# oviniciuscesar/Pseudo-Quadrature-Mirror-Filter

Measured on NVIDIA B200. Metric: PQMF analyze+inverse throughput (n_band=16), higher is better.
Workload: dtype f32

## Files before the change

pseudo-quadrature-mirror-filter_b200/csrc/hankel4.cuh:

```cuda
#pragma once
#include <cuda_fp16.h>
#include <cuda_runtime.h>
#include <math.h>
#include <stdint.h>
#include <string.h>

#include <atomic>

#include "half_io.cuh"
#include "hankel16.cuh"
#include "pcm.cuh"
#include "ptx.cuh"

namespace pqmf {

constexpr int kH4Workers = 256;
constexpr int kH4Threads = kH4Workers + 32;
constexpr int kH4SynWorkers = 288;
constexpr int kH4SynThreads = kH4SynWorkers + 32;
constexpr int kH4Rows = 128;
constexpr int kH4TileSamples = 64 * kH4Rows;
constexpr int kH4MaxPlaneRows = 144;
constexpr float kH4Res = 2048.0f;

// ... 39 lines not shown
  constexpr uint32_t idesc128 = ptx::umma_idesc_f16(m, 128), idesc64 = ptx::umma_idesc_f16(m, 64);
  constexpr uint32_t kStep = 2 * kBankRows;
  auto a_step = [&](int s) {
    const uint32_t byte = 32u * (uint32_t)s + (uint32_t)pad_bytes;
    return (uint64_t)(8u * (byte >> 7) + ((byte >> 4) & 7u));
  };
  auto mma = [&](uint32_t d, uint64_t a, uint64_t bdesc, uint32_t idesc, bool acc) {
    if constexpr (PAIR) ptx::umma_pair_f16(d, a, bdesc, idesc, acc);
    else ptx::umma_f16(d, a, bdesc, idesc, acc);
  };
  for (int s = tlo; s < ks - thi; ++s) mma(d_tmem, da1 + a_step(s), db + (uint64_t)(kStep * s), idesc128, s != tlo);
  for (int s = 0; s < tlo; ++s) mma(d_tmem, da1 + a_step(s), db64 + (uint64_t)(kStep * s), idesc64, true);
  for (int s = ks - thi; s < ks; ++s) mma(d_tmem, da1 + a_step(s), db64 + (uint64_t)(kStep * s), idesc64, true);
  for (int s = tlo; s < ks - thi; ++s) mma(d_tmem + 64u, da2 + a_step(s), db64 + (uint64_t)(kStep * s), idesc64, true);
}

__device__ __forceinline__ void split2_f16s(float a, float b, uint32_t& h1_bits, uint32_t& h2_bits) {
  const __half2 h1 = __floats2half2_rn(a, b);
  const float2 h1f = __half22float2(h1);
  const float2 r = __ffma2_rn(h1f, make_float2(-kH4Res, -kH4Res), __fmul2_rn(make_float2(a, b), make_float2(kH4Res, kH4Res)));
  const __half2 h2 = __floats2half2_rn(r.x, r.y);
  h1_bits = *reinterpret_cast<const uint32_t*>(&h1);
  h2_bits = *reinterpret_cast<const uint32_t*>(&h2);
}
__device__ __forceinline__ float2 h4_combine2(uint32_t d0a, uint32_t d0b, uint32_t d1a, uint32_t d1b) {
  const float2 t = __ffma2_rn(make_float2(__uint_as_float(d1a), __uint_as_float(d1b)), make_float2(1.0f / kH4Res, 1.0f / kH4Res),
                              make_float2(__uint_as_float(d0a), __uint_as_float(d0b)));
  constexpr float kInv = 1.0f / (float)(1 << kH16ScaleLog2);
  return __fmul2_rn(t, make_float2(kInv, kInv));
}

template <int N>
__device__ __forceinline__ void h4_tmem_ld(uint32_t taddr, uint32_t (&r)[N]) {
  static_assert(N == 2 || N == 4 || N == 8 || N == 16 || N == 32, "columns per load");
  if constexpr (N == 2) ptx::tmem_ld2(taddr, r);
  else if constexpr (N == 4) ptx::tmem_ld4(taddr, r);
  else if constexpr (N == 8) ptx::tmem_ld8(taddr, r);
  else if constexpr (N == 16) ptx::tmem_ld16(taddr, r);
  else ptx::tmem_ld32(taddr, r);
}

__device__ __forceinline__ void h4_split_store8(const float (&w)[8], unsigned char* p1, int plane, uint32_t off) {
  uint4 a, bq;
  split2_f16s(w[0], w[1], a.x, bq.x);
  split2_f16s(w[2], w[3], a.y, bq.y);
  split2_f16s(w[4], w[5], a.z, bq.z);
  split2_f16s(w[6], w[7], a.w, bq.w);
  unsigned char* p2 = p1 + plane;
  *reinterpret_cast<uint4*>(p1 + off) = a;
  *reinterpret_cast<uint4*>(p2 + off) = bq;
}

__device__ __forceinline__ void h4_synthesis_chunk8(const float4 (&v)[8], int j, uint32_t fl, float (&w)[8]) {
#pragma unroll
  for (int kk = 0; kk < 8; ++kk) {
    const float t = j == 0 ? v[kk].x : j == 1 ? v[kk].y : j == 2 ? v[kk].z : v[kk].w;
    w[kk] = (kk & 1) ? __uint_as_float(__float_as_uint(t) ^ fl) : t;
  }
}

template <int M>
__device__ __forceinline__ void h4_drain_analysis(uint32_t tmem, int dbuf, int tid, int first, int parity, float (&v)[64 / M][M / 2]) {
  constexpr int FR = 64 / M, HB = M / 2;
  const uint32_t taddr = tmem + ((uint32_t)(((tid >> 5) & 3) * 32) << 16) + (uint32_t)(dbuf * 128 + HB * (tid >> 7));
  uint32_t r0[FR][HB], r1[FR][HB];
#pragma unroll
  for (int dl = 0; dl < FR; ++dl) {
    h4_tmem_ld<HB>(taddr + dl * M, r0[dl]);
    h4_tmem_ld<HB>(taddr + 64 + dl * M, r1[dl]);
  }
  ptx::tmem_ld_wait();
#pragma unroll
  for (int dl = 0; dl < FR; ++dl) {
    const uint32_t flip = (((FR > 1 ? dl : first) + parity) & 1) == 0 ? 0x80000000u : 0u;
#pragma unroll
    for (int kk = 0; kk < HB; kk += 2) {
      const float2 t = h4_combine2(r0[dl][kk], r0[dl][kk + 1], r1[dl][kk], r1[dl][kk + 1]);
      v[dl][kk] = t.x;
      v[dl][kk + 1] = __uint_as_float(__float_as_uint(t.y) ^ flip);
    }
  }
}

__device__ __forceinline__ void h4_drain_synthesis(uint32_t tmem, int dbuf, int tid, float (&val)[4][8]) {
  const int hb = tid >> 7, lane = tid & 31;
  const uint32_t taddr = tmem + ((uint32_t)(((tid >> 5) & 3) * 32) << 16) + (uint32_t)(dbuf * 128 + 2 * hb * 16);
  uint32_t r0[2][16], r1[2][16];
  ptx::tmem_ld16(taddr, r0[0]);
  ptx::tmem_ld16(taddr + 64, r1[0]);
  ptx::tmem_ld16(taddr + 16, r0[1]);
  ptx::tmem_ld16(taddr + 80, r1[1]);
  ptx::tmem_ld_wait();
#pragma unroll
  for (int q = 0; q < 4; ++q)
#pragma unroll
    for (int e = 0; e < 8; e += 2) {
      const int c0 = 8 * (q & 1) + e;
      const float2 t = h4_combine2(r0[q >> 1][c0], r0[q >> 1][c0 + 1], r1[q >> 1][c0], r1[q >> 1][c0 + 1]);
      val[q][e] = t.x;
      val[q][e + 1] = t.y;
    }
  const bool b0 = lane & 1, b1 = lane & 2;
#pragma unroll
  for (int pr = 0; pr < 2; ++pr)
#pragma unroll
    for (int e = 0; e < 8; ++e) {
      const float recv = __shfl_xor_sync(0xffffffffu, b0 ? val[2 * pr][e] : val[2 * pr + 1][e], 1);
      val[2 * pr + 1][e] = b0 ? val[2 * pr + 1][e] : recv;
      val[2 * pr][e] = b0 ? recv : val[2 * pr][e];
    }
#pragma unroll
  for (int u = 0; u < 2; ++u)
#pragma unroll
    for (int e = 0; e < 8; ++e) {
      const float recv = __shfl_xor_sync(0xffffffffu, b1 ? val[u][e] : val[u + 2][e], 2);
      val[u + 2][e] = b1 ? val[u + 2][e] : recv;
      val[u][e] = b1 ? recv : val[u][e];
    }
}

#ifdef PQMF_H4_TRACE
#define H4_TRACE_PARAM , long long* trace
#define H4_TRACE(x) , x
#define H4_STAMP(k) do { if (trace && blockIdx.x == 0 && (tid & 31) == 0 && it < 64) trace[((size_t)it * 8 + (tid >> 5)) * 8 + (k)] = clock64(); } while (0)
#else
#define H4_TRACE_PARAM
#define H4_TRACE(x)
#define H4_STAMP(k) do { } while (0)
#endif

struct H4Smem {
  unsigned char *bank, *planes;
  uint64_t *pfull, *mma_bar, *bankfull;
  uint32_t* tmem_slot;
};
__device__ __forceinline__ H4Smem h4_carve(unsigned char* smem, const H4Shape& g) {
  H4Smem s;
  s.bank = smem;
  s.planes = smem + g.bank;
  s.pfull = reinterpret_cast<uint64_t*>(smem + g.bank + 4 * g.plane);
  s.mma_bar = s.pfull + 2;
  s.bankfull = s.mma_bar + 2;
  s.tmem_slot = reinterpret_cast<uint32_t*>(s.bankfull + 1);
  return s;
}

template <bool PAIR>
__device__ __forceinline__ uint32_t h4_prologue(const H4Smem& s, const H4Shape& g, const uint16_t* bank_images, uint32_t rank, int worker_warps,
                                                int tid) {
  const int warp = tid >> 5;
  ptx::grid_dep_launch();
  if (tid == 0) {
    for (int i = 0; i < 2; ++i) {
      ptx::mbar_init(&s.pfull[i], worker_warps * (PAIR ? 2 : 1));
      ptx::mbar_init(&s.mma_bar[i], 1);
    }
    ptx::mbar_init(s.bankfull, 1);
    ptx::fence_barrier_init();
    ptx::mbar_arrive_expect_tx(s.bankfull, (uint32_t)g.bank);
    ptx::bulk_g2s(s.bank, reinterpret_cast<const unsigned char*>(bank_images) + (size_t)rank * g.bank, (uint32_t)g.bank, s.bankfull);
  }
  if (warp == 0) {
    if constexpr (PAIR) {
      ptx::tmem_alloc_pair(s.tmem_slot, 256);
    } else {
      ptx::tmem_alloc(s.tmem_slot, 256);
      ptx::tmem_relinquish();
    }
  }
  ptx::tc_fence_before();
  __syncthreads();
  if constexpr (PAIR) ptx::cluster_sync_all();
  ptx::tc_fence_after();
  ptx::grid_dep_wait();
  return *s.tmem_slot;
}

template <bool PAIR>
__device__ __forceinline__ void h4_teardown(uint32_t tmem, int warp) {
  ptx::tc_fence_before();
  __syncthreads();
  if constexpr (PAIR) {
    ptx::cluster_sync_all();
    if (warp == 0) ptx::tmem_dealloc_pair(tmem, 256);
  } else {
    if (warp == 0) ptx::tmem_dealloc(tmem, 256);
  }
}

template <bool PAIR>
__device__ __forceinline__ void h4_issuer_loop(const H4Smem& s, const H4Shape& g, uint32_t tmem, unsigned n_iter, int pad_bytes, int tlo,
                                               int thi) {
  const uint32_t bank_addr = ptx::smem_u32(s.bank), plane_addr = ptx::smem_u32(s.planes);
  for (unsigned it = 0; it < n_iter; ++it) {
    const int pb = (int)(it & 1);
    ptx::mbar_wait(&s.pfull[pb], (it >> 1) & 1);
    ptx::tc_fence_after();
    if (ptx::elect_one_sync()) {
      h4_issue_mmas<PAIR>(tmem + (uint32_t)(pb * 128), plane_addr + (2 * pb) * g.plane, plane_addr + (2 * pb + 1) * g.plane, bank_addr, g.ks,
                          pad_bytes, tlo, thi);
// ... 296 lines not shown
    const int n_fq = (g.rows * FR + FPI - 1) / FPI;
    const int bg = tid / n_fq, fq = tid - bg * n_fq;
    const bool has_item = tid < n_fq * NBG;
    float4 v0[8];
    auto load4h = [&](const uint16_t* at, bool ok) {
      if (!ok) return make_float4(0.f, 0.f, 0.f, 0.f);
      const float2 raw = ptx::ldg64_na(at);
      return make_float4(raw.x, raw.y, 0.f, 0.f);
    };
    auto load_frames = [&](unsigned bb, unsigned cc, unsigned hh) {
      if (p.reverse && bb < n_rows) {
        bb = n_rows - 1 - bb;
        cc = tpr - 1 - cc;
      }
      const long n = (long)cc * (kH4Rows * FR) + nbase + FPI * fq;
      const bool live = bb < n_rows && has_item;
      const size_t row = (size_t)bb * G + hh;
      if constexpr (HALF) {
        if constexpr (M >= 8) {
          const uint16_t* sp = reinterpret_cast<const uint16_t*>(p.s) + (row * M + 8 * bg) * p.F + n;
          const bool ok = live && n >= 0 && n + 3 < p.F;
#pragma unroll
          for (int kk = 0; kk < 8; ++kk) v0[kk] = load4h(sp + (size_t)kk * p.F, ok);
        } else {
          const uint16_t* sp = reinterpret_cast<const uint16_t*>(p.s) + row * M * p.F + n;
#pragma unroll
          for (int kk = 0; kk < 8; ++kk) {
            const int b4 = kk >> 1, hf = kk & 1;
            v0[kk] = load4h(sp + (size_t)b4 * p.F + 4 * hf, live && n + 4 * hf >= 0 && n + 4 * hf + 3 < p.F);
          }
        }
      } else if constexpr (M >= 8) {
        const float* sp = p.s + (row * M + 8 * bg) * p.F + n;
        const bool ok = live && n >= 0 && n + 3 < p.F;
#pragma unroll
        for (int kk = 0; kk < 8; ++kk) v0[kk] = ok ? ptx::ldg128_na(reinterpret_cast<const float4*>(sp + (size_t)kk * p.F)) : make_float4(0.f, 0.f, 0.f, 0.f);
      } else {
        const float* sp = p.s + row * M * p.F + n;
#pragma unroll
        for (int kk = 0; kk < 8; ++kk) {
          const int b4 = kk >> 1, hf = kk & 1;
          const bool ok = live && n + 4 * hf >= 0 && n + 4 * hf + 3 < p.F;
          v0[kk] = ok ? ptx::ldg128_na(reinterpret_cast<const float4*>(sp + (size_t)b4 * p.F + 4 * hf)) : make_float4(0.f, 0.f, 0.f, 0.f);
        }
      }
    };
    const uint32_t flip_even = (p.parity & 1) ? 0u : 0x80000000u, flip_odd = flip_even ^ 0x80000000u;
    auto convert = [&](int pb) {
      float4 v[8];
#pragma unroll
      for (int kk = 0; kk < 8; ++kk) v[kk] = HALF ? h4_widen4<IO>(v0[kk]) : v0[kk];
      if (!has_item) return;
      unsigned char* p1 = sm.planes + (2 * pb) * g.plane;
#pragma unroll
      for (int j = 0; j < 4; ++j) {
        float w[8];
        uint32_t o;
        if constexpr (M >= 8) {
          h4_synthesis_chunk8(v, j, (j & 1) ? flip_odd : flip_even, w);
          o = sw128_offset((uint32_t)(4 * fq + j) * (2u * M) + 16u * bg);
        } else {
#pragma unroll
          for (int kk = 0; kk < 8; ++kk) {
            const int b4 = kk & 3, odd = kk >> 2;
            const float4& q = v[2 * b4 + (j >> 1)];
            const int cmp = 2 * (j & 1) + odd;
            const float t = cmp == 0 ? q.x : cmp == 1 ? q.y : cmp == 2 ? q.z : q.w;
            w[kk] = (b4 & 1) ? __uint_as_float(__float_as_uint(t) ^ (odd ? flip_odd : flip_even)) : t;
          }
          o = sw128_offset((uint32_t)(8 * fq + 2 * j) * (2u * M));
        }
        h4_split_store8(w, p1, g.plane, o);
      }
    };
    uint32_t held[4][4];
    auto drain = [&](int dbuf) {
      if (warp >= 8 || prev_b >= n_rows) return;
      unsigned bb = prev_b, cc = prev_c;
      if (p.reverse) {
        bb = n_rows - 1 - bb;
        cc = tpr - 1 - cc;
      }
      const size_t row = (size_t)bb * G + prev_h;
      const int i = tid & 127, hb = tid >> 7, lane = tid & 31;
      float val[4][8];
      h4_drain_synthesis(tmem, dbuf, tid, val);
      const long total = p.F * M;
      const long t0 = (long)cc * kH4TileSamples + 64 * (i & ~3) + 32 * hb + 8 * (lane & 3);
      if constexpr (PCM) {
        if (G == 2) {
#pragma unroll
          for (int q = 0; q < 4; ++q) {
            uint32_t w[4];
#pragma unroll
            for (int k = 0; k < 4; ++k)
              w[k] = (uint32_t)(uint16_t)pcm_quantise(val[q][2 * k]) | ((uint32_t)(uint16_t)pcm_quantise(val[q][2 * k + 1]) << 16);
            if (prev_h == 0) {
#pragma unroll
              for (int k = 0; k < 4; ++k) held[q][k] = w[k];
            } else if (t0 + 64 * q + 7 < total) {
              float lr[8];
#pragma unroll
              for (int k = 0; k < 4; ++k) {
                lr[2 * k] = __uint_as_float(__byte_perm(held[q][k], w[k], 0x5410));
                lr[2 * k + 1] = __uint_as_float(__byte_perm(held[q][k], w[k], 0x7632));
              }
              ptx::stg256_cs(reinterpret_cast<float*>(p.pcm_out + ((size_t)bb * total + t0 + 64 * q) * 2), lr);
            }
          }
          return;
        }
#pragma unroll
        for (int q = 0; q < 4; ++q)
          if (t0 + 64 * q + 7 < total) pcm_store8(p.pcm_out, p.C, (long)row, t0 + 64 * q, total, val[q]);
        return;
      }
      if constexpr (HALF) {
        uint16_t* op = reinterpret_cast<uint16_t*>(p.out) + row * total + t0;
#pragma unroll
        for (int q = 0; q < 4; ++q)
          if (t0 + 64 * q + 7 < total) {
            const uint4 w = make_uint4(h4_narrow2<IO>(val[q][0], val[q][1]), h4_narrow2<IO>(val[q][2], val[q][3]), h4_narrow2<IO>(val[q][4], val[q][5]),
                                       h4_narrow2<IO>(val[q][6], val[q][7]));
            __stcs(reinterpret_cast<uint4*>(op + (size_t)q * 64), w);
          }
        return;
      }
      float* op = p.out + row * total + t0;
#pragma unroll
      for (int q = 0; q < 4; ++q)
        if (t0 + 64 * q + 7 < total) {
          if (p.accumulate) {
            float prev[8];
            ptx::ldg256_cs(op + (size_t)q * 64, prev);
#pragma unroll
            for (int e = 0; e < 8; ++e) val[q][e] += prev[e];
          }
          ptx::stg256_cs(op + (size_t)q * 64, val[q]);
        }
    };

    load_frames(b, c, h);
    h4_worker_loop<PAIR>(sm, pfull_leader, n_iter, tid, convert, [&] { load_frames(b1, c1, h1); }, drain, [&] {
      prev_b = b;
      prev_c = c;
      prev_h = h;
      b = b1;
      c = c1;
      h = h1;
      next_visit(b1, c1, h1);
    } H4_TRACE(p.trace));
  } H4_TRACE(p.trace));
}

struct H4Configured {
  std::atomic<int> bytes[64];
  H4Configured() {
    for (auto& b : bytes) b.store(0, std::memory_order_relaxed);
  }
};
inline int h4_sm_count(int dev) {
  static std::atomic<int> sm_count[64];
  int n = sm_count[dev].load(std::memory_order_relaxed);
  if (n == 0) {
    cudaDeviceGetAttribute(&n, cudaDevAttrMultiProcessorCount, dev);
    n = n > 0 ? n : 148;
    sm_count[dev].store(n, std::memory_order_relaxed);
  }
  return n;
}
template <typename Kern>
inline int h4_configure(Kern kern, int bytes, H4Configured& configured, int& sm_count_out) {
  int dev = 0;
  cudaGetDevice(&dev);
  dev &= 63;
  if (configured.bytes[dev].load(std::memory_order_acquire) < bytes) {
    cudaError_t e = cudaFuncSetAttribute(kern, cudaFuncAttributeMaxDynamicSharedMemorySize, bytes);
    if (e != cudaSuccess) return (int)e;
    int seen = configured.bytes[dev].load(std::memory_order_relaxed);
    while (seen < bytes && !configured.bytes[dev].compare_exchange_weak(seen, bytes, std::memory_order_release)) {
    }
  }
  sm_count_out = h4_sm_count(dev);
  return 0;
}

template <typename Params>
inline bool h4_set_tiles(Params& p, int B, long row_samples) {
  p.tiles_per_row = (row_samples + kH4TileSamples - 1) / kH4TileSamples;
  p.n_tiles = p.tiles_per_row * B;
  return p.tiles_per_row < (1L << 31) && p.n_tiles < (1L << 40);
}

template <bool PAIR, typename Kern, typename Params>
inline int h4_launch(Kern kern, const Params& p, int threads, H4Configured& configured, cudaStream_t st) {
  int sms = 0;
  if (!h4_shape_fits(p.g)) return -2;
  if (int e = h4_configure(kern, p.g.bytes, configured, sms)) return e;
  long grid = PAIR ? (sms & ~1) : sms;
  const long want = PAIR ? ((p.n_tiles + 1) & ~1L) : p.n_tiles;
  if (grid > want) grid = want;
  if constexpr (PAIR) {
    cudaLaunchConfig_t cfg = {};
    cfg.gridDim = dim3((unsigned)grid);
    cfg.blockDim = dim3((unsigned)threads);
    cfg.dynamicSmemBytes = (size_t)p.g.bytes;
    cfg.stream = st;
    cudaLaunchAttribute attr[2];
    attr[0].id = cudaLaunchAttributeClusterDimension;
    attr[0].val.clusterDim.x = 2;
    attr[0].val.clusterDim.y = 1;
    attr[0].val.clusterDim.z = 1;
    attr[1].id = cudaLaunchAttributeProgrammaticStreamSerialization;
    attr[1].val.programmaticStreamSerializationAllowed = 1;
    cfg.attrs = attr;
    cfg.numAttrs = 2;
    return (int)cudaLaunchKernelEx(&cfg, kern, p);
  } else {
    kern<<<(unsigned)grid, threads, p.g.bytes, st>>>(p);
    return (int)cudaGetLastError();
  }
}

template <int M, bool PAIR>
int h4_launch_analysis(H4AnalysisParams p, int B, cudaStream_t st, H4Io io = H4Io::F32) {
  static H4Configured configured[4];
  if (!h4_set_tiles(p, B, p.F * M)) return -2;
  if (p.in.pcm != nullptr) io = H4Io::PCM;
  if (io != H4Io::F32) {
    if constexpr (PAIR) {
      switch (io) {
        case H4Io::PCM: return h4_launch<PAIR>(h4_analysis_kernel<M, PAIR, H4Io::PCM>, p, kH4Threads, configured[1], st);
        case H4Io::F16: return h4_launch<PAIR>(h4_analysis_kernel<M, PAIR, H4Io::F16>, p, kH4Threads, configured[2], st);
        case H4Io::BF16: return h4_launch<PAIR>(h4_analysis_kernel<M, PAIR, H4Io::BF16>, p, kH4Threads, configured[3], st);
        default: return -2;
      }
    } else {
      return -2;
    }
  }
  return h4_launch<PAIR>(h4_analysis_kernel<M, PAIR, H4Io::F32>, p, kH4Threads, configured[0], st);
}

template <int M, bool PAIR>
int h4_launch_synthesis(H4SynthesisParams p, int B, cudaStream_t st, H4Io io = H4Io::F32) {
  static H4Configured configured[4];
  if (p.pcm_out != nullptr) {
    if constexpr (PAIR) {
      p.duo = (p.C == 2 && B % 2 == 0) ? 1 : 0;
      if (!h4_set_tiles(p, p.duo ? B / 2 : B, p.F * M)) return -2;
      return h4_launch<PAIR>(h4_synthesis_kernel<M, PAIR, H4Io::PCM>, p, kH4SynThreads, configured[1], st);
    } else {
      return -2;
    }
  }
  if (!h4_set_tiles(p, B, p.F * M)) return -2;
  if (h4_io_half(io)) {
    if constexpr (PAIR) {
      if (io == H4Io::F16) return h4_launch<PAIR>(h4_synthesis_kernel<M, PAIR, H4Io::F16>, p, kH4SynThreads, configured[2], st);
      return h4_launch<PAIR>(h4_synthesis_kernel<M, PAIR, H4Io::BF16>, p, kH4SynThreads, configured[3], st);
    } else {
      return -2;
    }
  }
  return h4_launch<PAIR>(h4_synthesis_kernel<M, PAIR, H4Io::F32>, p, kH4SynThreads, configured[0], st);
}

inline void hankel4_build_banks(const float* hk , int M, int L, int jlo, int kt, uint16_t* img_analysis, uint16_t* img_synthesis) {
  auto bits = [](float v) {
    const __half h = __float2half_rn(v);
    uint16_t u;
    memcpy(&u, &h, 2);
    return u;
  };
  const int ks = (kt + 64 - M + 15) / 16, kp = 16 * ks;
  const int elo = jlo / M, ehi = (jlo + kt) / M - 1;
  const float sa = (float)(1 << kH16ScaleLog2), ss = (float)M * sa;
  for (int kc = 0; kc < kp / 8; ++kc)
    for (int row = 0; row < 128; ++row)
      for (int e8 = 0; e8 < 8; ++e8) {
        const int kap = 8 * kc + e8;
        const int part = row / 64, delta = (row % 64) / M, q = row % M;
        const size_t at = ((size_t)kc * 128 + row) * 8 + e8;
        {
          const int j = kap - M * delta;
          const float v = (j >= 0 && j < kt && jlo + j < L) ? sa * hk[(size_t)q * L + jlo + j] : 0.f;
          const float c1 = __half2float(__float2half_rn(v));
          img_analysis[at] = part == 0 ? bits(c1) : bits((v - c1) * kH4Res);
        }
        {
          const int e = kap / M, kb = kap % M, lag = delta + ehi - e;
          const float v = (lag >= elo && lag <= ehi && M * lag + q < L) ? ss * hk[(size_t)kb * L + M * lag + q] : 0.f;
          const float c1 = __half2float(__float2half_rn(v));
          img_synthesis[at] = part == 0 ? bits(c1) : bits((v - c1) * kH4Res);
        }
      }
}

inline void hankel4_pair_image(const uint16_t* single , int ks, uint16_t* pair ) {
  const int chunks = 2 * ks;
  for (int r = 0; r < 2; ++r)
    for (int kc = 0; kc < chunks; ++kc)
      for (int row = 0; row < 96; ++row) {
        const int src = row < 64 ? 64 * r + row : 32 * r + (row - 64);
        memcpy(pair + (((size_t)r * chunks + kc) * 96 + row) * 8, single + ((size_t)kc * 128 + src) * 8, 16);
      }
}

inline int hankel4_pick_trim(const float* hk , int M, int L, int jlo, int kt, bool synthesis, double budget, int max_trim = 7) {
  const int ks = (kt + 64 - M + 15) / 16, fr = 64 / M, elo = jlo / M, ehi = (jlo + kt) / M - 1;
  int best = 0;
  for (int trim = 1; trim <= max_trim && ks - 2 * trim >= 1; ++trim) {
    double worst = 0.0;
    for (int delta = 0; delta < fr; ++delta)
      for (int q = 0; q < M; ++q) {
        double sum = 0.0;
        for (int side = 0; side < 2; ++side)
          for (int t = 0; t < trim; ++t) {
            const int s = side ? ks - 1 - t : t;
            for (int e16 = 0; e16 < 16; ++e16) {
              const int kap = 16 * s + e16;
              if (!synthesis) {
                const int j = kap - M * delta;
                if (j >= 0 && j < kt && jlo + j < L) sum += fabs((double)hk[(size_t)q * L + jlo + j]);
              } else {
                const int e = kap / M, kb = kap % M, lag = delta + ehi - e;
                if (lag >= elo && lag <= ehi && M * lag + q < L) sum += (double)M * fabs((double)hk[(size_t)kb * L + M * lag + q]);
              }
            }
          }
        worst = sum > worst ? sum : worst;
      }
    if (2.0 * worst / 2048.0 <= budget) best = trim;
    else break;
  }
  return best;
}

}
```

pseudo-quadrature-mirror-filter_b200/csrc/hankel4_stream.cuh:

```cuda
#pragma once
#include <type_traits>

#include "hankel4.cuh"
#include "stream_pool.cuh"

namespace pqmf {

struct H4StreamGeom {
  int rows_b;
  int hrows;
  int pitch;
  int spt;
};
inline H4StreamGeom h4_stream_geom(long block_samples, int hist_samples) {
  H4StreamGeom s;
  s.rows_b = (int)(block_samples / 64);
  s.hrows = hist_samples / 64;
  s.pitch = (s.rows_b + s.hrows + 3) & ~3;
  s.spt = kH4Rows / s.pitch;
  return s;
}

struct H4AnalysisStreamParams {
  const float* x;
// ... 195 lines not shown
    const int tid = threadIdx.x, warp = tid >> 5;
    for (int u = sg.spt * sg.pitch * 32 + tid; u < g.rows * 32; u += kH4SynWorkers)
#pragma unroll
      for (int pl = 0; pl < 4; ++pl) reinterpret_cast<float*>(sm.planes + pl * g.plane)[u] = 0.f;
    const int n_fq = sg.spt * sg.pitch * FR / 4;
    const int bg = tid / n_fq, wq = tid - bg * n_fq;
    const bool has_item = tid < NBG * n_fq;
    const int region_frames = sg.pitch * FR, hist_fr = sg.hrows * FR, block_fr = sg.rows_b * FR;
    const int lt = (4 * wq) / region_frames, lf = 4 * wq - lt * region_frames;
    const int fb = lf - hist_fr;
    constexpr int kDead = 1 << 20;
    const size_t band0 = ((size_t)blockIdx.x * sg.spt + lt) * M + 8 * bg;
    const size_t step_state = (size_t)gridDim.x * sg.spt * M * p.K;
    int slot = kDead;
    const float* src = p.s;
    size_t src_step = 0, src_pitch = 0;
    float* roll = nullptr;
    int hofs = -1, rofs = -1;
    if (has_item) {
      if (fb < 0) {
        slot = lt;
        if constexpr (POOL) {
          hofs = 8 * bg * p.K + (p.K - hist_fr) + lf;
        } else {
          src = p.state_in + band0 * p.K + (p.K - hist_fr) + lf;
          src_step = step_state;
        }
        src_pitch = (size_t)p.K;
      } else if (fb < block_fr) {
        slot = lt;
        src = p.s + band0 * p.F + fb;
        src_step = (size_t)gridDim.x * sg.spt * M * p.F;
        src_pitch = (size_t)p.F;
        if (fb >= p.F - p.K) {
          if constexpr (POOL) rofs = 8 * bg * p.K + (fb - (p.F - p.K));
          else roll = p.state_out + band0 * p.K + (fb - (p.F - p.K));
        }
      }
    }
    float4 v[8];
    int nlive = 0;
    uint32_t flip_ld = 0;
    auto load_tile = [&](long tile) {
      nlive = (int)min((long)sg.spt, (long)p.B - tile * sg.spt);
      if constexpr (POOL) {
        int id = slot < nlive ? __ldg(p.pool.ids + tile * sg.spt + slot) : -1;
        if ((unsigned)id >= (unsigned)p.pool.P) id = -1;
        const int ph = id >= 0 ? __ldg(p.pool.phase + id) : 0;
        const size_t row = ((size_t)(ph & 1) * p.pool.P + (size_t)id) * M * p.K;
        const float* from = hofs >= 0 ? p.state_in + row + hofs : src;
#pragma unroll
        for (int kk = 0; kk < 8; ++kk)
          v[kk] = id >= 0 ? ptx::ldg128_na(reinterpret_cast<const float4*>(from + (size_t)kk * src_pitch)) : make_float4(0.f, 0.f, 0.f, 0.f);
        src += src_step;
        roll = (rofs >= 0 && id >= 0) ? p.state_out + ((size_t)(~ph & 1) * p.pool.P + (size_t)id) * M * p.K + rofs : nullptr;
        flip_ld = (ph & 2) ? 0u : 0x80000000u;
      } else {
        const bool live = slot < nlive;
#pragma unroll
        for (int kk = 0; kk < 8; ++kk)
          v[kk] = live ? ptx::ldg128_na(reinterpret_cast<const float4*>(src + (size_t)kk * src_pitch)) : make_float4(0.f, 0.f, 0.f, 0.f);
        src += src_step;
      }
    };
    const uint32_t flip_even = (p.parity & 1) ? 0u : 0x80000000u, flip_odd = flip_even ^ 0x80000000u;
    auto convert = [&](int pb) {
      if (!has_item) return;
      unsigned char* p1 = sm.planes + (2 * pb) * g.plane;
      const uint32_t fe = POOL ? flip_ld : flip_even, fo = POOL ? flip_ld ^ 0x80000000u : flip_odd;
      if (roll != nullptr) {
        if (POOL || slot < nlive) {
#pragma unroll
          for (int kk = 0; kk < 8; ++kk) *reinterpret_cast<float4*>(roll + (size_t)kk * p.K) = v[kk];
        }
        if constexpr (!POOL) roll += step_state;
      }
#pragma unroll
      for (int j = 0; j < 4; ++j) {
        float w[8];
        h4_synthesis_chunk8(v, j, (j & 1) ? fo : fe, w);
        h4_split_store8(w, p1, g.plane, sw128_offset((uint32_t)(4 * wq + j) * (2u * M) + 16u * bg));
      }
    };
    const int i = tid & 127, hb = tid >> 7, lane = tid & 31;
    const int i0 = i & ~3, et = i0 / sg.pitch, eq0 = i0 - et * sg.pitch;
    const bool e_rows = et < sg.spt && eq0 < sg.rows_b;
    float* orun = p.out + ((size_t)blockIdx.x * sg.spt + et) * (size_t)(p.F * M) + 64 * eq0 + 32 * hb + 8 * (lane & 3);
    const size_t out_step = (size_t)gridDim.x * sg.spt * (size_t)(p.F * M);
    long tile = blockIdx.x, prev_tile = 0;
    auto drain = [&](int dbuf) {
      if (warp >= 8) return;
      float val[4][8];
      h4_drain_synthesis(tmem, dbuf, tid, val);
      float* op = orun;
      orun += out_step;
      if (!e_rows || prev_tile * sg.spt + et >= p.B) return;
#pragma unroll
      for (int q = 0; q < 4; ++q) ptx::stg256_cs(op + (size_t)q * 64, val[q]);
    };

    load_tile(tile);
    h4_worker_loop<true>(sm, pfull_leader, n_iter, tid, convert, [&] { load_tile(tile + gridDim.x); }, drain, [&] {
      prev_tile = tile;
      tile += gridDim.x;
    } H4_TRACE(nullptr));
  } H4_TRACE(nullptr));
}

template <int M, typename Params>
inline int h4_launch_analysis_stream(Params p, cudaStream_t st) {
  constexpr bool POOL = std::is_same_v<Params, H4AnalysisStreamPoolParams>;
  static H4Configured configured;
  p.n_tiles = (p.B + p.s.spt - 1) / p.s.spt;
  return h4_launch<true>(h4_analysis_stream_kernel<M, POOL>, p, kH4Threads, configured, st);
}
template <int M, typename Params>
inline int h4_launch_synthesis_stream(Params p, cudaStream_t st) {
  constexpr bool POOL = std::is_same_v<Params, H4SynthesisStreamPoolParams>;
  static H4Configured configured;
  p.n_tiles = (p.B + p.sg.spt - 1) / p.sg.spt;
  return h4_launch<true>(h4_synthesis_stream_kernel<M, POOL>, p, kH4SynThreads, configured, st);
}

}
```

pseudo-quadrature-mirror-filter_b200/csrc/ptx.cuh:

```cuda
#pragma once
#include <cuda_fp16.h>
#include <cuda_runtime.h>
#include <stdint.h>

namespace pqmf {
namespace ptx {

__device__ __forceinline__ uint32_t smem_u32(const void* p) { return (uint32_t)__cvta_generic_to_shared(p); }

__device__ __forceinline__ void mbar_init(uint64_t* bar, uint32_t count) {
  asm volatile("mbarrier.init.shared::cta.b64 [%0], %1;" ::"r"(smem_u32(bar)), "r"(count));
}
__device__ __forceinline__ void fence_barrier_init() { asm volatile("fence.mbarrier_init.release.cluster;" ::: "memory"); }
__device__ __forceinline__ void mbar_arrive_expect_tx(uint64_t* bar, uint32_t bytes) {
  asm volatile("mbarrier.arrive.expect_tx.shared::cta.b64 _, [%0], %1;" ::"r"(smem_u32(bar)), "r"(bytes) : "memory");
}
__device__ __forceinline__ void mbar_arrive(uint64_t* bar) {
  asm volatile("mbarrier.arrive.shared::cta.b64 _, [%0];" ::"r"(smem_u32(bar)) : "memory");
}
__device__ __forceinline__ bool mbar_try_wait(uint64_t* bar, uint32_t parity) {
  uint32_t ok;
  asm volatile(
      "{\n\t.reg .pred p;\n\t"
      "mbarrier.try_wait.parity.shared::cta.b64 p, [%1], %2, %3;\n\t"
// ... 26 lines not shown
__device__ __forceinline__ void fence_proxy_async() { asm volatile("fence.proxy.async.shared::cta;" ::: "memory"); }

__device__ __forceinline__ bool elect_one_sync() {
  uint32_t pred;
  asm volatile(
      "{\n\t.reg .pred p;\n\t"
      "elect.sync _|p, 0xffffffff;\n\t"
      "selp.u32 %0, 1, 0, p;\n\t}"
      : "=r"(pred));
  return pred != 0;
}

__device__ __forceinline__ void tmem_alloc(uint32_t* dst_smem, uint32_t ncols) {
  asm volatile("tcgen05.alloc.cta_group::1.sync.aligned.shared::cta.b32 [%0], %1;" ::"r"(smem_u32(dst_smem)), "r"(ncols) : "memory");
}
__device__ __forceinline__ void tmem_relinquish() { asm volatile("tcgen05.relinquish_alloc_permit.cta_group::1.sync.aligned;" ::: "memory"); }
__device__ __forceinline__ void tmem_dealloc(uint32_t taddr, uint32_t ncols) {
  asm volatile("tcgen05.dealloc.cta_group::1.sync.aligned.b32 %0, %1;" ::"r"(taddr), "r"(ncols) : "memory");
}
__device__ __forceinline__ void tc_fence_before() { asm volatile("tcgen05.fence::before_thread_sync;" ::: "memory"); }
__device__ __forceinline__ void tc_fence_after() { asm volatile("tcgen05.fence::after_thread_sync;" ::: "memory"); }

__device__ __forceinline__ uint64_t umma_desc(uint32_t smem_addr, uint32_t lbo_bytes, uint32_t sbo_bytes) {
  uint64_t d = 0;
  d |= (uint64_t)((smem_addr & 0x3FFFFu) >> 4);
  d |= (uint64_t)((lbo_bytes >> 4) & 0x3FFFu) << 16;
  d |= (uint64_t)((sbo_bytes >> 4) & 0x3FFFu) << 32;
  d |= (uint64_t)1 << 46;
  return d;
}
__host__ __device__ constexpr uint32_t umma_idesc_tf32(int m, int n) {
  return (1u << 4) | (2u << 7) | (2u << 10) | ((uint32_t)(n >> 3) << 17) | ((uint32_t)(m >> 4) << 24);
}
__host__ __device__ constexpr uint32_t umma_idesc_f16(int m, int n) {
  return (1u << 4) | (0u << 7) | (0u << 10) | ((uint32_t)(n >> 3) << 17) | ((uint32_t)(m >> 4) << 24);
}
__device__ __forceinline__ void umma_f16(uint32_t d_tmem, uint64_t a_desc, uint64_t b_desc, uint32_t idesc, bool accumulate) {
  asm volatile(
      "{\n\t.reg .pred p;\n\t"
      "setp.ne.b32 p, %4, 0;\n\t"
      "tcgen05.mma.cta_group::1.kind::f16 [%0], %1, %2, %3, p;\n\t}" ::"r"(d_tmem),
      "l"(a_desc), "l"(b_desc), "r"(idesc), "r"((uint32_t)accumulate)
      : "memory");
}
__device__ __forceinline__ void umma_tf32(uint32_t d_tmem, uint64_t a_desc, uint64_t b_desc, uint32_t idesc, bool accumulate) {
  asm volatile(
      "{\n\t.reg .pred p;\n\t"
      "setp.ne.b32 p, %4, 0;\n\t"
      "tcgen05.mma.cta_group::1.kind::tf32 [%0], %1, %2, %3, p;\n\t}" ::"r"(d_tmem),
      "l"(a_desc), "l"(b_desc), "r"(idesc), "r"((uint32_t)accumulate)
      : "memory");
}
__device__ __forceinline__ void umma_commit(uint64_t* bar) {
  asm volatile("tcgen05.commit.cta_group::1.mbarrier::arrive::one.shared::cluster.b64 [%0];" ::"r"(smem_u32(bar)) : "memory");
}
__device__ __forceinline__ void tmem_ld16(uint32_t taddr, uint32_t (&r)[16]) {
  asm volatile(
      "tcgen05.ld.sync.aligned.32x32b.x16.b32 {%0,%1,%2,%3,%4,%5,%6,%7,%8,%9,%10,%11,%12,%13,%14,%15}, [%16];"
      : "=r"(r[0]), "=r"(r[1]), "=r"(r[2]), "=r"(r[3]), "=r"(r[4]), "=r"(r[5]), "=r"(r[6]), "=r"(r[7]), "=r"(r[8]), "=r"(r[9]),
        "=r"(r[10]), "=r"(r[11]), "=r"(r[12]), "=r"(r[13]), "=r"(r[14]), "=r"(r[15])
      : "r"(taddr)
      : "memory");
}
__device__ __forceinline__ void tmem_ld2(uint32_t taddr, uint32_t (&r)[2]) {
  asm volatile("tcgen05.ld.sync.aligned.32x32b.x2.b32 {%0,%1}, [%2];" : "=r"(r[0]), "=r"(r[1]) : "r"(taddr) : "memory");
}
__device__ __forceinline__ void tmem_ld4(uint32_t taddr, uint32_t (&r)[4]) {
  asm volatile("tcgen05.ld.sync.aligned.32x32b.x4.b32 {%0,%1,%2,%3}, [%4];" : "=r"(r[0]), "=r"(r[1]), "=r"(r[2]), "=r"(r[3]) : "r"(taddr) : "memory");
}
__device__ __forceinline__ void tmem_ld8(uint32_t taddr, uint32_t (&r)[8]) {
  asm volatile("tcgen05.ld.sync.aligned.32x32b.x8.b32 {%0,%1,%2,%3,%4,%5,%6,%7}, [%8];"
               : "=r"(r[0]), "=r"(r[1]), "=r"(r[2]), "=r"(r[3]), "=r"(r[4]), "=r"(r[5]), "=r"(r[6]), "=r"(r[7])
               : "r"(taddr)
               : "memory");
}
__device__ __forceinline__ void tmem_ld32(uint32_t taddr, uint32_t (&r)[32]) {
  asm volatile(
      "tcgen05.ld.sync.aligned.32x32b.x32.b32 {%0,%1,%2,%3,%4,%5,%6,%7,%8,%9,%10,%11,%12,%13,%14,%15,"
      "%16,%17,%18,%19,%20,%21,%22,%23,%24,%25,%26,%27,%28,%29,%30,%31}, [%32];"
      : "=r"(r[0]), "=r"(r[1]), "=r"(r[2]), "=r"(r[3]), "=r"(r[4]), "=r"(r[5]), "=r"(r[6]), "=r"(r[7]), "=r"(r[8]), "=r"(r[9]),
        "=r"(r[10]), "=r"(r[11]), "=r"(r[12]), "=r"(r[13]), "=r"(r[14]), "=r"(r[15]), "=r"(r[16]), "=r"(r[17]), "=r"(r[18]),
        "=r"(r[19]), "=r"(r[20]), "=r"(r[21]), "=r"(r[22]), "=r"(r[23]), "=r"(r[24]), "=r"(r[25]), "=r"(r[26]), "=r"(r[27]),
        "=r"(r[28]), "=r"(r[29]), "=r"(r[30]), "=r"(r[31])
      : "r"(taddr)
      : "memory");
}
__device__ __forceinline__ void tmem_ld_wait() { asm volatile("tcgen05.wait::ld.sync.aligned;" ::: "memory"); }

__device__ __forceinline__ uint32_t cluster_ctarank() {
  uint32_t r;
  asm volatile("mov.u32 %0, %%cluster_ctarank;" : "=r"(r));
  return r;
}
__device__ __forceinline__ void cluster_sync_all() {
  asm volatile("barrier.cluster.arrive.release.aligned;" ::: "memory");
  asm volatile("barrier.cluster.wait.acquire.aligned;" ::: "memory");
}
__device__ __forceinline__ uint32_t mapa_shared(uint32_t local_smem_addr, uint32_t rank) {
  uint32_t r;
  asm volatile("mapa.shared::cluster.u32 %0, %1, %2;" : "=r"(r) : "r"(local_smem_addr), "r"(rank));
  return r;
}
__device__ __forceinline__ void mbar_arrive_cluster(uint32_t cluster_addr) {
  asm volatile("mbarrier.arrive.shared::cluster.b64 _, [%0];" ::"r"(cluster_addr) : "memory");
}
__device__ __forceinline__ void mbar_wait_cluster(uint64_t* bar, uint32_t parity) {
  const uint32_t addr = smem_u32(bar);
  uint32_t done = 0;
  while (!done) {
    asm volatile(
        "{\n\t.reg .pred p;\n\t"
        "mbarrier.try_wait.parity.acquire.cluster.shared::cta.b64 p, [%1], %2;\n\t"
        "selp.u32 %0, 1, 0, p;\n\t}"
        : "=r"(done)
        : "r"(addr), "r"(parity)
        : "memory");
  }
}
__device__ __forceinline__ void tmem_alloc_pair(uint32_t* slot, uint32_t cols) {
  asm volatile("tcgen05.alloc.cta_group::2.sync.aligned.shared::cta.b32 [%0], %1;" ::"r"(smem_u32(slot)), "r"(cols) : "memory");
  asm volatile("tcgen05.relinquish_alloc_permit.cta_group::2.sync.aligned;" ::: "memory");
}
__device__ __forceinline__ void tmem_dealloc_pair(uint32_t addr, uint32_t cols) {
  asm volatile("tcgen05.dealloc.cta_group::2.sync.aligned.b32 %0, %1;" ::"r"(addr), "r"(cols) : "memory");
}
__device__ __forceinline__ void umma_pair_f16(uint32_t d_tmem, uint64_t a_desc, uint64_t b_desc, uint32_t idesc, bool accumulate) {
  asm volatile(
      "{\n\t.reg .pred p;\n\t"
      "setp.ne.b32 p, %4, 0;\n\t"
      "tcgen05.mma.cta_group::2.kind::f16 [%0], %1, %2, %3, p;\n\t}" ::"r"(d_tmem),
      "l"(a_desc), "l"(b_desc), "r"(idesc), "r"((uint32_t)accumulate)
      : "memory");
}
__device__ __forceinline__ void umma_pair_commit(uint64_t* bar) {
  asm volatile("tcgen05.commit.cta_group::2.mbarrier::arrive::one.shared::cluster.multicast::cluster.b64 [%0], %1;" ::"r"(smem_u32(bar)),
               "h"((uint16_t)3)
               : "memory");
}

__device__ __forceinline__ void grid_dep_wait() { asm volatile("griddepcontrol.wait;" ::: "memory"); }
__device__ __forceinline__ void grid_dep_launch() { asm volatile("griddepcontrol.launch_dependents;" ::: "memory"); }

__device__ __forceinline__ void stg256_cs(float* p, const float (&v)[8]) {
  asm volatile("st.global.cs.v8.f32 [%0], {%1,%2,%3,%4,%5,%6,%7,%8};" ::"l"(p), "f"(v[0]), "f"(v[1]), "f"(v[2]), "f"(v[3]), "f"(v[4]),
               "f"(v[5]), "f"(v[6]), "f"(v[7])
               : "memory");
}
__device__ __forceinline__ void ldg256_cs(const float* p, float (&v)[8]) {
  asm volatile("ld.global.cs.v8.f32 {%0,%1,%2,%3,%4,%5,%6,%7}, [%8];"
               : "=f"(v[0]), "=f"(v[1]), "=f"(v[2]), "=f"(v[3]), "=f"(v[4]), "=f"(v[5]), "=f"(v[6]), "=f"(v[7])
               : "l"(p));
}

__device__ __forceinline__ void ldg256_na(const float* p, float (&v)[8]) {
  asm volatile("ld.global.nc.L1::no_allocate.v8.f32 {%0,%1,%2,%3,%4,%5,%6,%7}, [%8];"
               : "=f"(v[0]), "=f"(v[1]), "=f"(v[2]), "=f"(v[3]), "=f"(v[4]), "=f"(v[5]), "=f"(v[6]), "=f"(v[7])
               : "l"(p));
}
__device__ __forceinline__ float4 ldg128_na(const float4* p) {
  float4 v;
  asm volatile("ld.global.nc.L1::no_allocate.v4.f32 {%0,%1,%2,%3}, [%4];" : "=f"(v.x), "=f"(v.y), "=f"(v.z), "=f"(v.w) : "l"(p));
  return v;
}
__device__ __forceinline__ float2 ldg64_na(const void* p) {
  float2 v;
  asm volatile("ld.global.nc.L1::no_allocate.v2.f32 {%0,%1}, [%2];" : "=f"(v.x), "=f"(v.y) : "l"(p));
// ... 18 lines not shown
```

Baseline: 264,400.

## Permute synthesis matrix rows and use 16x256b TMEM loads to drop shuffle transpose

Synthesis weight rows are now permuted on the host so that the 16x256b tcgen05.ld shape delivers each thread the output samples it stores. This removes the two rounds of warp shuffles that previously transposed the drained values. Store addressing in both the tile and stream kernels is updated to match the new per-thread sample layout, with stride 512 between q groups and per-q row validity. The trade-off is less contiguous per-warp stores and extra per-q offset registers in the stream path.

Result: faster. 267,800, median of 6 (+1.3%).

```diff
diff --git a/pseudo-quadrature-mirror-filter_b200/csrc/hankel4.cuh b/pseudo-quadrature-mirror-filter_b200/csrc/hankel4.cuh
--- a/pseudo-quadrature-mirror-filter_b200/csrc/hankel4.cuh
+++ b/pseudo-quadrature-mirror-filter_b200/csrc/hankel4.cuh
@@ -145,40 +145,25 @@
   }
 }
 
+constexpr int h4_syn_sample(int c) { return (c & ~0x1e) | ((c >> 2) & 6) | ((c & 6) << 2); }
+
 __device__ __forceinline__ void h4_drain_synthesis(uint32_t tmem, int dbuf, int tid, float (&val)[4][8]) {
-  const int hb = tid >> 7, lane = tid & 31;
-  const uint32_t taddr = tmem + ((uint32_t)(((tid >> 5) & 3) * 32) << 16) + (uint32_t)(dbuf * 128 + 2 * hb * 16);
+  const int hb = tid >> 7;
+  const uint32_t taddr = tmem + ((uint32_t)(((tid >> 5) & 3) * 32) << 16) + (uint32_t)(dbuf * 128 + 32 * hb);
   uint32_t r0[2][16], r1[2][16];
-  ptx::tmem_ld16(taddr, r0[0]);
-  ptx::tmem_ld16(taddr + 64, r1[0]);
-  ptx::tmem_ld16(taddr + 16, r0[1]);
-  ptx::tmem_ld16(taddr + 80, r1[1]);
+  ptx::tmem_ld16x256b_x4(taddr, r0[0]);
+  ptx::tmem_ld16x256b_x4(taddr + 64, r1[0]);
+  ptx::tmem_ld16x256b_x4(taddr + (16u << 16), r0[1]);
+  ptx::tmem_ld16x256b_x4(taddr + (16u << 16) + 64, r1[1]);
   ptx::tmem_ld_wait();
 #pragma unroll
   for (int q = 0; q < 4; ++q)
 #pragma unroll
-    for (int e = 0; e < 8; e += 2) {
-      const int c0 = 8 * (q & 1) + e;
+    for (int r = 0; r < 4; ++r) {
+      const int c0 = 4 * r + 2 * (q & 1);
       const float2 t = h4_combine2(r0[q >> 1][c0], r0[q >> 1][c0 + 1], r1[q >> 1][c0], r1[q >> 1][c0 + 1]);
-      val[q][e] = t.x;
-      val[q][e + 1] = t.y;
-    }
-  const bool b0 = lane & 1, b1 = lane & 2;
-#pragma unroll
-  for (int pr = 0; pr < 2; ++pr)
-#pragma unroll
-    for (int e = 0; e < 8; ++e) {
-      const float recv = __shfl_xor_sync(0xffffffffu, b0 ? val[2 * pr][e] : val[2 * pr + 1][e], 1);
-      val[2 * pr + 1][e] = b0 ? val[2 * pr + 1][e] : recv;
-      val[2 * pr][e] = b0 ? recv : val[2 * pr][e];
-    }
-#pragma unroll
-  for (int u = 0; u < 2; ++u)
-#pragma unroll
-    for (int e = 0; e < 8; ++e) {
-      const float recv = __shfl_xor_sync(0xffffffffu, b1 ? val[u][e] : val[u + 2][e], 2);
-      val[u + 2][e] = b1 ? val[u + 2][e] : recv;
-      val[u][e] = b1 ? recv : val[u][e];
+      val[q][2 * r] = t.x;
+      val[q][2 * r + 1] = t.y;
     }
 }
 
@@ -641,11 +626,11 @@
         cc = tpr - 1 - cc;
       }
       const size_t row = (size_t)bb * G + prev_h;
-      const int i = tid & 127, hb = tid >> 7, lane = tid & 31;
+      const int hb = tid >> 7, lane = tid & 31;
       float val[4][8];
       h4_drain_synthesis(tmem, dbuf, tid, val);
       const long total = p.F * M;
-      const long t0 = (long)cc * kH4TileSamples + 64 * (i & ~3) + 32 * hb + 8 * (lane & 3);
+      const long t0 = (long)cc * kH4TileSamples + 64 * (32 * (warp & 3) + (lane >> 2)) + 32 * hb + 8 * (lane & 3);
       if constexpr (PCM) {
         if (G == 2) {
 #pragma unroll
@@ -657,45 +642,45 @@
             if (prev_h == 0) {
 #pragma unroll
               for (int k = 0; k < 4; ++k) held[q][k] = w[k];
-            } else if (t0 + 64 * q + 7 < total) {
+            } else if (t0 + 512 * q + 7 < total) {
               float lr[8];
 #pragma unroll
               for (int k = 0; k < 4; ++k) {
                 lr[2 * k] = __uint_as_float(__byte_perm(held[q][k], w[k], 0x5410));
                 lr[2 * k + 1] = __uint_as_float(__byte_perm(held[q][k], w[k], 0x7632));
               }
-              ptx::stg256_cs(reinterpret_cast<float*>(p.pcm_out + ((size_t)bb * total + t0 + 64 * q) * 2), lr);
+              ptx::stg256_cs(reinterpret_cast<float*>(p.pcm_out + ((size_t)bb * total + t0 + 512 * q) * 2), lr);
             }
           }
           return;
         }
 #pragma unroll
         for (int q = 0; q < 4; ++q)
-          if (t0 + 64 * q + 7 < total) pcm_store8(p.pcm_out, p.C, (long)row, t0 + 64 * q, total, val[q]);
+          if (t0 + 512 * q + 7 < total) pcm_store8(p.pcm_out, p.C, (long)row, t0 + 512 * q, total, val[q]);
         return;
       }
       if constexpr (HALF) {
         uint16_t* op = reinterpret_cast<uint16_t*>(p.out) + row * total + t0;
 #pragma unroll
         for (int q = 0; q < 4; ++q)
-          if (t0 + 64 * q + 7 < total) {
+          if (t0 + 512 * q + 7 < total) {
             const uint4 w = make_uint4(h4_narrow2<IO>(val[q][0], val[q][1]), h4_narrow2<IO>(val[q][2], val[q][3]), h4_narrow2<IO>(val[q][4], val[q][5]),
                                        h4_narrow2<IO>(val[q][6], val[q][7]));
-            __stcs(reinterpret_cast<uint4*>(op + (size_t)q * 64), w);
+            __stcs(reinterpret_cast<uint4*>(op + (size_t)q * 512), w);
           }
         return;
       }
       float* op = p.out + row * total + t0;
 #pragma unroll
       for (int q = 0; q < 4; ++q)
-        if (t0 + 64 * q + 7 < total) {
+        if (t0 + 512 * q + 7 < total) {
           if (p.accumulate) {
             float prev[8];
-            ptx::ldg256_cs(op + (size_t)q * 64, prev);
+            ptx::ldg256_cs(op + (size_t)q * 512, prev);
 #pragma unroll
             for (int e = 0; e < 8; ++e) val[q][e] += prev[e];
           }
-          ptx::stg256_cs(op + (size_t)q * 64, val[q]);
+          ptx::stg256_cs(op + (size_t)q * 512, val[q]);
         }
     };
 
@@ -848,8 +833,9 @@
           img_analysis[at] = part == 0 ? bits(c1) : bits((v - c1) * kH4Res);
         }
         {
-          const int e = kap / M, kb = kap % M, lag = delta + ehi - e;
-          const float v = (lag >= elo && lag <= ehi && M * lag + q < L) ? ss * hk[(size_t)kb * L + M * lag + q] : 0.f;
+          const int smp = h4_syn_sample(row % 64), dl = smp / M, ph = smp % M;
+          const int e = kap / M, kb = kap % M, lag = dl + ehi - e;
+          const float v = (lag >= elo && lag <= ehi && M * lag + ph < L) ? ss * hk[(size_t)kb * L + M * lag + ph] : 0.f;
           const float c1 = __half2float(__float2half_rn(v));
           img_synthesis[at] = part == 0 ? bits(c1) : bits((v - c1) * kH4Res);
         }
diff --git a/pseudo-quadrature-mirror-filter_b200/csrc/hankel4_stream.cuh b/pseudo-quadrature-mirror-filter_b200/csrc/hankel4_stream.cuh
--- a/pseudo-quadrature-mirror-filter_b200/csrc/hankel4_stream.cuh
+++ b/pseudo-quadrature-mirror-filter_b200/csrc/hankel4_stream.cuh
@@ -301,11 +301,17 @@
         h4_split_store8(w, p1, g.plane, sw128_offset((uint32_t)(4 * wq + j) * (2u * M) + 16u * bg));
       }
     };
-    const int i = tid & 127, hb = tid >> 7, lane = tid & 31;
-    const int i0 = i & ~3, et = i0 / sg.pitch, eq0 = i0 - et * sg.pitch;
-    const bool e_rows = et < sg.spt && eq0 < sg.rows_b;
-    float* orun = p.out + ((size_t)blockIdx.x * sg.spt + et) * (size_t)(p.F * M) + 64 * eq0 + 32 * hb + 8 * (lane & 3);
-    const size_t out_step = (size_t)gridDim.x * sg.spt * (size_t)(p.F * M);
+    const int hb = tid >> 7, lane = tid & 31;
+    const int block_out = (int)(p.F * M);
+    int et[4], oofs[4];
+#pragma unroll
+    for (int q = 0; q < 4; ++q) {
+      const int i = 32 * (warp & 3) + 8 * q + (lane >> 2), t = i / sg.pitch, eq = i - t * sg.pitch;
+      et[q] = t < sg.spt && eq < sg.rows_b ? t : kDead;
+      oofs[q] = t * block_out + 64 * eq + 32 * hb + 8 * (lane & 3);
+    }
+    float* orun = p.out + (size_t)blockIdx.x * sg.spt * (size_t)block_out;
+    const size_t out_step = (size_t)gridDim.x * sg.spt * (size_t)block_out;
     long tile = blockIdx.x, prev_tile = 0;
     auto drain = [&](int dbuf) {
       if (warp >= 8) return;
@@ -313,9 +319,10 @@
       h4_drain_synthesis(tmem, dbuf, tid, val);
       float* op = orun;
       orun += out_step;
-      if (!e_rows || prev_tile * sg.spt + et >= p.B) return;
-#pragma unroll
-      for (int q = 0; q < 4; ++q) ptx::stg256_cs(op + (size_t)q * 64, val[q]);
+      const long live = (long)p.B - prev_tile * sg.spt;
+#pragma unroll
+      for (int q = 0; q < 4; ++q)
+        if (et[q] < live) ptx::stg256_cs(op + oofs[q], val[q]);
     };
 
     load_tile(tile);
diff --git a/pseudo-quadrature-mirror-filter_b200/csrc/ptx.cuh b/pseudo-quadrature-mirror-filter_b200/csrc/ptx.cuh
--- a/pseudo-quadrature-mirror-filter_b200/csrc/ptx.cuh
+++ b/pseudo-quadrature-mirror-filter_b200/csrc/ptx.cuh
@@ -132,6 +132,14 @@
         "=r"(r[10]), "=r"(r[11]), "=r"(r[12]), "=r"(r[13]), "=r"(r[14]), "=r"(r[15]), "=r"(r[16]), "=r"(r[17]), "=r"(r[18]),
         "=r"(r[19]), "=r"(r[20]), "=r"(r[21]), "=r"(r[22]), "=r"(r[23]), "=r"(r[24]), "=r"(r[25]), "=r"(r[26]), "=r"(r[27]),
         "=r"(r[28]), "=r"(r[29]), "=r"(r[30]), "=r"(r[31])
+      : "r"(taddr)
+      : "memory");
+}
+__device__ __forceinline__ void tmem_ld16x256b_x4(uint32_t taddr, uint32_t (&r)[16]) {
+  asm volatile(
+      "tcgen05.ld.sync.aligned.16x256b.x4.b32 {%0,%1,%2,%3,%4,%5,%6,%7,%8,%9,%10,%11,%12,%13,%14,%15}, [%16];"
+      : "=r"(r[0]), "=r"(r[1]), "=r"(r[2]), "=r"(r[3]), "=r"(r[4]), "=r"(r[5]), "=r"(r[6]), "=r"(r[7]), "=r"(r[8]), "=r"(r[9]),
+        "=r"(r[10]), "=r"(r[11]), "=r"(r[12]), "=r"(r[13]), "=r"(r[14]), "=r"(r[15])
       : "r"(taddr)
       : "memory");
 }
```
